# wen-yuan-zhang/MaterialRefGS

Measured on AMD Instinct MI355X. Metric: full-render fwd+bwd views/sec at 800x800/300k surfels; grad max-rel-err vs ref, higher is better.
Workload: dtype f32; 1 GPU; C3 shell scene through render_surfel: P=300000, 800x800, S=8 + deferred BRDF shading, fwd+bwd; P=300000, H=800, W=800, S=8, sh_degree=3, num_rendered=1153468, cameras_cycled=2, parallelism=single GPU, glue_epilogue=True

## Files before the change

### materialrefgs_amd/csrc/mrgs_render_bwd.hip

```cpp
#include "mrgs_blend_math.h"

#ifndef MRGS_BWD_STAGES
#define MRGS_BWD_STAGES 1
#endif


__device__ __forceinline__ void swap32_add(float& a, float b)
{
    typedef unsigned u2 __attribute__((ext_vector_type(2)));
    const u2 r = __builtin_amdgcn_permlane32_swap(__float_as_uint(a), __float_as_uint(b), false, false);
    a = __uint_as_float(r.x) + __uint_as_float(r.y);
}
__device__ __forceinline__ void swap16_add(float& a, float b)
{
    typedef unsigned u2 __attribute__((ext_vector_type(2)));
    const u2 r = __builtin_amdgcn_permlane16_swap(__float_as_uint(a), __float_as_uint(b), false, false);
    a = __uint_as_float(r.x) + __uint_as_float(r.y);
}

__device__ __forceinline__ float rows_reduce4(float a0, float a1, float a2, float a3)
{
    float t0, t1, u;
    asm volatile(
        "s_nop 1\n\t"
        "v_add_f32_dpp %0, %3, %3 row_ror:8 row_mask:0xf bank_mask:0xf\n\t"
        "v_add_f32_dpp %1, %5, %5 row_ror:8 row_mask:0xf bank_mask:0xf\n\t"
        "v_add_f32_dpp %0, %4, %4 row_ror:8 row_mask:0xf bank_mask:0xc\n\t"
        "v_add_f32_dpp %1, %6, %6 row_ror:8 row_mask:0xf bank_mask:0xc\n\t"
        "s_nop 0\n\t"
        "v_add_f32_dpp %2, %0, %0 row_half_mirror row_mask:0xf bank_mask:0xf\n\t"
        "v_add_f32_dpp %2, %1, %1 row_half_mirror row_mask:0xf bank_mask:0xa\n\t"
        "s_nop 1\n\t"
        "v_add_f32_dpp %2, %2, %2 quad_perm:[2,3,0,1] row_mask:0xf bank_mask:0xf\n\t"
        "s_nop 1\n\t"
        "v_add_f32_dpp %2, %2, %2 quad_perm:[1,0,3,2] row_mask:0xf bank_mask:0xf\n\t"
        : "=&v"(t0), "=&v"(t1), "=&v"(u)
        : "v"(a0), "v"(a1), "v"(a2), "v"(a3));
    return u;
}
__device__ __forceinline__ float rows_reduce2(float a0, float a1)
{
    float t;
    asm volatile(
        "s_nop 1\n\t"
        "v_add_f32_dpp %0, %1, %1 row_ror:8 row_mask:0xf bank_mask:0xf\n\t"
        "v_add_f32_dpp %0, %2, %2 row_ror:8 row_mask:0xf bank_mask:0xc\n\t"
        "s_nop 1\n\t"
        "v_add_f32_dpp %0, %0, %0 row_half_mirror row_mask:0xf bank_mask:0xf\n\t"
        "s_nop 1\n\t"
        "v_add_f32_dpp %0, %0, %0 quad_perm:[2,3,0,1] row_mask:0xf bank_mask:0xf\n\t"
        "s_nop 1\n\t"
        "v_add_f32_dpp %0, %0, %0 quad_perm:[1,0,3,2] row_mask:0xf bank_mask:0xf\n\t"
        : "=&v"(t)
        : "v"(a0), "v"(a1));
    return t;
}
__device__ __forceinline__ float rows_reduce1(float v)
{
    v = mrgs_dpp_add<0x128, 0xf>(v);
    v = mrgs_dpp_add<0x124, 0xf>(v);
    v = mrgs_dpp_add<0x122, 0xf>(v);
    v = mrgs_dpp_add<0x121, 0xf>(v);
    return v;
}

struct ReduceLane { uint32_t off16, off8, off4; bool w16, w8, w4; };
__device__ __forceinline__ ReduceLane mrgs_reduce_lane(int lane)
{
    const int row = lane >> 4, bank = (lane >> 2) & 3;
    const int sub = ((row & 1) << 1) | (row >> 1);
    ReduceLane r;
    r.off16 = 4u * (uint32_t)(8 * (bank & 1) + 4 * (bank >> 1) + sub);
    r.off8 = 4u * (uint32_t)(4 * (bank >> 1) + sub);
    r.off4 = 4u * (uint32_t)sub;
    r.w16 = (lane & 3) == 0;
    r.w8 = (lane & 7) == 0;
    r.w4 = (lane & 15) == 0;
    return r;
}

__device__ __forceinline__ void atomic_add_at(float* __restrict__ base, uint32_t byte_off, float v)
{
    atomicAdd((float*)((char*)base + byte_off), v);
}

template <int K>
__device__ __forceinline__ void wave_reduce_atomic_add(float (&v)[K], float* __restrict__ base, uint32_t row_off, const ReduceLane& rl)
{
    static_assert(K % 4 == 0, "pad the value count to a multiple of 4");
#pragma unroll
    for (int i = 0; i < K / 2; i++) swap32_add(v[2 * i], v[2 * i + 1]);
#pragma unroll
    for (int i = 0; i < K / 4; i++) swap16_add(v[4 * i], v[4 * i + 2]);
    constexpr int N4 = K / 4;
    constexpr int NB4 = N4 / 4;
    constexpr int REM = N4 - 4 * NB4;
#pragma unroll
    for (int t = 0; t < NB4; t++) {
        const float u = rows_reduce4(v[16 * t], v[16 * t + 4], v[16 * t + 8], v[16 * t + 12]);
        if (rl.w16) atomic_add_at(base, row_off + (64u * t + rl.off16), u);
    }
    if (REM >= 2) {
        const float u = rows_reduce2(v[16 * NB4], v[16 * NB4 + 4]);
        if (rl.w8) atomic_add_at(base, row_off + (64u * NB4 + rl.off8), u);
    }
    if (REM == 1 || REM == 3) {
        constexpr int vbase = 16 * NB4 + (REM == 3 ? 8 : 0);
        const float u = rows_reduce1(v[vbase]);
        if (rl.w4) atomic_add_at(base, row_off + (4u * vbase + rl.off4), u);
    }
}

__device__ __forceinline__ void wave_reduce_atomic_add2(float a, float b, float* __restrict__ base, uint32_t byte_off, int lane)
{
    swap32_add(a, b);
    a = rows_reduce1(a);
    a += __int_as_float(__builtin_amdgcn_update_dpp(0, __float_as_int(a), 0x142, 0xa, 0xf, false));
    if ((lane & 31) == 16) atomic_add_at(base, byte_off + 4u * (uint32_t)(lane >> 5), a);
}

__device__ __forceinline__ void wave_reduce_atomic_add1(float a, float* __restrict__ base, uint32_t byte_off, int lane)
{
    float z = 0.0f;
    swap32_add(a, z);
    a = rows_reduce1(a);
    a += __int_as_float(__builtin_amdgcn_update_dpp(0, __float_as_int(a), 0x142, 0xa, 0xf, false));
    if (lane == 16) atomic_add_at(base, byte_off, a);
}

#ifdef MRGS_WAVE_STATS
__device__ unsigned long long g_wave_stats[8 * 65536];
extern "C" int mrgs_wave_stats(unsigned long long* host, int n)
{
    return (int)hipMemcpyFromSymbol(host, HIP_SYMBOL(g_wave_stats), sizeof(unsigned long long) * n);
}
#define WS_ENTRY() const unsigned long long ws_te = wall_clock64(); unsigned long long ws_dbg[3];
#define WS_DBG , ws_dbg
#define WS_BEGIN() const unsigned long long ws_t0 = wall_clock64(), ws_c0 = __builtin_amdgcn_s_memtime(); unsigned ws_iters = 0, ws_act = 0, ws_chunks = 0;
#define WS_ITER(a) { ws_iters++; ws_act += (a) ? 1 : 0; }
#define WS_CHUNK() ws_chunks++;
#define WS_END() if (lane == 0 && b < 65536) { unsigned long long* w = g_wave_stats + 8 * (size_t)b; w[6] = ((ws_dbg[0] - ws_te) << 40) | ((ws_dbg[2] - ws_te) << 16) | ws_dbg[1]; w[7] = ws_te; w[0] = ws_t0; w[1] = wall_clock64(); \
        w[2] = __builtin_amdgcn_s_memtime() - ws_c0; w[3] = ((unsigned long long)ws_iters << 32) | ws_act; w[4] = ((unsigned long long)ws_chunks << 32) | (unsigned)max_contrib; \
        w[5] = (unsigned long long)__builtin_amdgcn_s_getreg((4 << 0) | (0 << 6) | (31 << 11)) | ((unsigned long long)__builtin_amdgcn_s_getreg((20 << 0) | (0 << 6) | (31 << 11)) << 32); }
#else
#define WS_ENTRY()
#define WS_DBG
#define WS_BEGIN()
#define WS_ITER(a)
#define WS_CHUNK()
#define WS_END()
#endif

#ifndef MRGS_BWD_WPE0
#define MRGS_BWD_WPE0 5
#endif
#ifndef MRGS_BWD_WPE8
#define MRGS_BWD_WPE8 4
#endif
template <int S_MAX, bool FV, int S_LIVE>
__global__ void __launch_bounds__(64) __attribute__((amdgpu_waves_per_eu(S_MAX == 0 ? MRGS_BWD_WPE0 : S_MAX <= 8 ? MRGS_BWD_WPE8 : 2, 8))) render_bwd_kernel(
    const uint2* __restrict__ ranges, const uint32_t* __restrict__ bwd_assign, uint32_t* __restrict__ q_bwd, const uint32_t* __restrict__ cu_state, const uint32_t* __restrict__ point_list,
    const uint8_t* __restrict__ cflag, int S, int W, int H, int tiles_x, int ntiles,
    const float4* __restrict__ rec, const float* __restrict__ features, const float* __restrict__ bg,
    const float* __restrict__ final_Ts, const uint32_t* __restrict__ n_contrib, const float* __restrict__ dL_dpixels,
    const float* __restrict__ dL_dpixels_f, const float* __restrict__ dL_dothers, float* __restrict__ grad_rec, int gstride, int slots)
{
    constexpr int SF = S_MAX > 0 ? S_MAX : 1;
    constexpr bool XREC = S_LIVE > S_MAX;
    static_assert(!XREC || (S_MAX == 8 && S_LIVE == 9 && FV), "one record channel: rows of twelve floats, eight staged");
    constexpr int S_ROW = XREC ? 12 : S_MAX;
    constexpr int S_STAGED = S_LIVE < S_MAX ? S_LIVE : S_MAX;
    constexpr int SFA = S_LIVE > SF ? S_LIVE : SF;
    constexpr int K = 16 + S_LIVE;
    constexpr int KT = K & ~3;
    __shared__ StageBuf<SF> stage[MRGS_BWD_STAGES];

    const int lane = threadIdx.x;
    const int b = blockIdx.x;
    WS_ENTRY();
    const uint32_t item = mrgs_pull_item(q_bwd, cu_state, bwd_assign, ntiles, b & 7, b >> 3, lane, slots WS_DBG);
    if (item == 0xFFFFFFFFu) return;
    const int tile = (int)((item & 0x1FFFFFFFu) >> 2), quad = (int)(item & 3u);
    const uint32_t prio = (item >> 29) & 3u;
    const uint2 range = ranges[tile];
    const int tx = tile % tiles_x, ty = tile / tiles_x;
    const int bx = tx * 2 + (quad & 1), by = ty * 2 + (quad >> 1);
    const int pxi = bx * 8 + (lane & 7), pyi = by * 8 + (lane >> 3);
    const bool inside = pxi < W && pyi < H;
    const float px = (float)pxi, py = (float)pyi;
    const int HW = H * W;
    const int pix = inside ? W * pyi + pxi : 0;

    const int last_contributor = inside ? (int)n_contrib[pix] : 0;
    int max_contrib = last_contributor;
#pragma unroll
    for (int d = 32; d >= 1; d >>= 1) max_contrib = max(max_contrib, __shfl_xor(max_contrib, d, 64));
    if (max_contrib == 0) return;
    WS_BEGIN();
    if (prio == 3u) __builtin_amdgcn_s_setprio(3);
    else if (prio == 2u) __builtin_amdgcn_s_setprio(2);
    else if (prio == 1u) __builtin_amdgcn_s_setprio(1);
    const int median_contributor = inside ? (int)n_contrib[pix + HW] : 0;

    const float T_final = inside ? final_Ts[pix] : 0.f;
    float T = T_final;
    float dL_dpixel[3] = {0.f, 0.f, 0.f};
    float dL_dpixel_f[SFA];
#pragma unroll
    for (int i = 0; i < SFA; i++) dL_dpixel_f[i] = 0.f;
    float accum_dot = 0.f;
    float dL_dreg = 0.f, dL_ddepth = 0.f, dL_daccum = 0.f, dL_dnormal2D[3] = {0.f, 0.f, 0.f}, dL_dmedian_depth = 0.f;
    if (inside && last_contributor > 0) {
        dL_ddepth = dL_dothers[0 * HW + pix];
        dL_daccum = dL_dothers[1 * HW + pix];
        dL_dnormal2D[0] = dL_dothers[2 * HW + pix];
        dL_dnormal2D[1] = dL_dothers[3 * HW + pix];
        dL_dnormal2D[2] = dL_dothers[4 * HW + pix];
        dL_dmedian_depth = dL_dothers[5 * HW + pix];
        dL_dreg = dL_dothers[6 * HW + pix];
#pragma unroll
        for (int i = 0; i < 3; i++) dL_dpixel[i] = dL_dpixels[i * HW + pix];
        if (S_MAX > 0) {
#pragma unroll
            for (int i = 0; i < S_LIVE; i++)
                if (i < S) dL_dpixel_f[i] = dL_dpixels_f[(size_t)i * HW + pix];
        }
    }
    const float final_D = inside ? final_Ts[pix + HW] : 0.f;
    const float final_D2 = inside ? final_Ts[pix + 2 * HW] : 0.f;
    const float mscale = MRGS_FAR_N / (MRGS_FAR_N - MRGS_NEAR_N);
    const float dmd_scale = (MRGS_FAR_N * MRGS_NEAR_N) / (MRGS_FAR_N - MRGS_NEAR_N);
    const float bg_dot_dpixel = fmaf(bg[2], dL_dpixel[2], fmaf(bg[1], dL_dpixel[1], bg[0] * dL_dpixel[0]));

    const uint32_t* plist = point_list + range.x;
    const uint8_t* qm = cflag + (size_t)range.x * 4 + quad;
    const ReduceLane rl = mrgs_reduce_lane(lane);
    const uint32_t row_bytes = (uint32_t)gstride * 4u;
    const int c_top = (max_contrib - 1) / MRGS_CHUNK;
    uint32_t idq1 = 0, idq2 = 0;
    uint64_t mask_cur, exact_cur;
    {
        uint32_t id0 = 0, q0 = 0;
        if (c_top * MRGS_CHUNK + lane < max_contrib) { id0 = plist[c_top * MRGS_CHUNK + lane]; q0 = qm[(size_t)(c_top * MRGS_CHUNK + lane) * 4]; }
        if (c_top >= 1) idq1 = plist[(c_top - 1) * MRGS_CHUNK + lane] | ((uint32_t)qm[(size_t)((c_top - 1) * MRGS_CHUNK + lane) * 4] << 28);
        if (c_top >= 2) idq2 = plist[(c_top - 2) * MRGS_CHUNK + lane] | ((uint32_t)qm[(size_t)((c_top - 2) * MRGS_CHUNK + lane) * 4] << 28);
        const bool cand0 = q0 & 1u;
        mask_cur = __builtin_amdgcn_ballot_w64(cand0);
        exact_cur = __builtin_amdgcn_ballot_w64((q0 & 2u) != 0u);
        mrgs_stage_async<S_MAX, SF, FV, S_LIVE, S_ROW>(stage[c_top % MRGS_BWD_STAGES], rec, features, S, id0, cand0);
        if (cand0) stage[c_top % MRGS_BWD_STAGES].id[lane] = id0 * row_bytes;
    }

    for (int c = c_top; c >= 0; c--) {
        const int base = c * MRGS_CHUNK;
        mrgs_stage_wait();
        WS_CHUNK();
        uint64_t mask_nxt = 0ull, exact_nxt = 0ull;
        auto stage_next = [&]() {
            const bool cand1 = (idq1 >> 28) & 1u;
            exact_nxt = __builtin_amdgcn_ballot_w64(((idq1 >> 29) & 1u) != 0u);
            const uint32_t id1 = idq1 & 0x0FFFFFFFu;
            mask_nxt = __builtin_amdgcn_ballot_w64(cand1);
            mrgs_stage_async<S_MAX, SF, FV, S_LIVE, S_ROW>(stage[(c + 1) % MRGS_BWD_STAGES], rec, features, S, id1, cand1);
            if (cand1) stage[(c + 1) % MRGS_BWD_STAGES].id[lane] = id1 * row_bytes;
            idq1 = idq2;
            idq2 = 0;
            if (c >= 3) idq2 = plist[(c - 3) * MRGS_CHUNK + lane] | ((uint32_t)qm[(size_t)((c - 3) * MRGS_CHUNK + lane) * 4] << 28);
        };
        if (MRGS_BWD_STAGES == 2) stage_next();

        uint64_t mask = mask_cur;
        const uint64_t exact_mask = exact_cur;
        const StageBuf<SF>& sb = stage[c % MRGS_BWD_STAGES];

        auto blend_entry = [&](const SurfelGeom& sg, int j) {
            const int contributor = base + j;
            Hit h;
            bool active;
            active = mrgs_intersect(sg, px, py, h) & !(h.depth < MRGS_NEAR_LO);
            if (__builtin_expect((exact_mask >> j) & 1ull, 0)) active = mrgs_intersect_exact<true>(sg, px, py, h);
            active = active & inside & (contributor < last_contributor);
            const uint64_t amask = __builtin_amdgcn_ballot_w64(active);
            WS_ITER(amask != 0ull);
            if (amask == 0ull) return;
            const bool use3d = h.use3d;
            const bool a3 = active & use3d;
            const float4 a0 = sb.rec[3][j], a1 = sb.rec[4][j];
            const float normal[3] = {a0.x, a0.y, a0.z};
            const float col[3] = {a0.w, a1.x, a1.y};
            const float alpha = active ? h.alpha : 0.0f;
            const float G = active ? h.G : 0.0f;
            const float c_d = active ? h.depth : 1.0f;
            const float sx = a3 ? h.sx : 0.0f, sy = a3 ? h.sy : 0.0f;
            const float inv_pz = a3 ? h.inv_pz : 0.0f;

            float g[K];
            const float inv_1ma = mrgs_rcp(1.0f - alpha);
            T = T * inv_1ma;
            const float w = alpha * T;
            const float one_m_a = 1.0f - alpha;
            float q = 0.0f;
#pragma unroll
            for (int ch = 0; ch < 3; ch++) {
                q = fmaf(col[ch], dL_dpixel[ch], q);
                g[MRGS_G_COL + ch] = w * dL_dpixel[ch];
            }
            if (S_MAX > 0) {
#pragma unroll
                for (int ch = 0; ch < S_STAGED; ch++) {
                    const float f = (FV || ch < S) ? mrgs_staged_feature<FV>(sb, ch, j) : 0.0f;
                    q = fmaf(f, dL_dpixel_f[ch], q);
                    g[MRGS_G_FEAT + ch] = w * dL_dpixel_f[ch];
                }
                if (XREC) {
                    q = fmaf(a1.w, dL_dpixel_f[S_MAX], q);
                    g[MRGS_G_FEAT + S_MAX] = w * dL_dpixel_f[S_MAX];
                }
            }
#pragma unroll
            for (int ch = 0; ch < 3; ch++) {
                q = fmaf(normal[ch], dL_dnormal2D[ch], q);
                g[MRGS_G_NRM + ch] = w * dL_dnormal2D[ch];
            }
            const float inv_cd = mrgs_rcp(c_d);
            const float m_d = mscale * (1.0f - MRGS_NEAR_N * inv_cd);
            const float dmd_dd = dmd_scale * inv_cd * inv_cd;
            float dL_dz = (active & (contributor == median_contributor - 1)) ? dL_dmedian_depth : 0.0f;
            const float final_A = 1.0f - T_final;
            const float dL_dweight = fmaf(-2.0f * m_d, final_D, fmaf(m_d * m_d, final_A, final_D2)) * dL_dreg;
            const float dL_dmd = 2.0f * w * fmaf(m_d, final_A, -final_D) * dL_dreg;
            dL_dz = fmaf(dL_dmd, dmd_dd, dL_dz);
            q = fmaf(c_d, dL_ddepth, q);
            q += dL_daccum;
            q += dL_dweight;
            float dL_dalpha = q - accum_dot;
            accum_dot = fmaf(alpha, q, one_m_a * accum_dot);
            dL_dalpha *= T;
            dL_dalpha = fmaf(-T_final * inv_1ma, bg_dot_dpixel, dL_dalpha);
            dL_dalpha = active ? dL_dalpha : 0.0f;
            const float dL_dG = sg.g2.w * dL_dalpha;
            dL_dz = fmaf(w, dL_ddepth, dL_dz);
            {
                const float Twx = sg.g1.z, Twy = sg.g1.w;
                const float dGn = dL_dG * -G;
                const float dL_dsx = fmaf(dGn, sx, dL_dz * Twx);
                const float dL_dsy = fmaf(dGn, sy, dL_dz * Twy);
                const float dpx = dL_dsx * inv_pz, dpy = dL_dsy * inv_pz;
                const float dpz = -fmaf(dpx, sx, dpy * sy);
                const float ndkx = fmaf(-h.ly, dpz, h.lz * dpy);
                const float ndky = fmaf(-h.lz, dpx, h.lx * dpz);
                const float ndkz = fmaf(-h.lx, dpy, h.ly * dpx);
                const float ndlx = fmaf(-dpy, h.kz, dpz * h.ky);
                const float ndly = fmaf(-dpz, h.kx, dpx * h.kz);
                const float ndlz = fmaf(-dpx, h.ky, dpy * h.kx);
                g[0] = ndkx; g[1] = ndky; g[2] = ndkz;
                g[3] = ndlx; g[4] = ndly; g[5] = ndlz;
                g[6] = fmaf(px, -ndkx, fmaf(py, -ndlx, dL_dz * sx));
                g[7] = fmaf(px, -ndky, fmaf(py, -ndly, dL_dz * sy));
                g[8] = fmaf(px, -ndkz, fmaf(py, -ndlz, dL_dz));
            }
            g[MRGS_G_OPA] = G * dL_dalpha;
            const uint32_t row_off = sb.id[j];
            if constexpr (KT == K) {
                wave_reduce_atomic_add<K>(g, grad_rec, row_off, rl);
            } else {
                float gt[KT];
#pragma unroll
                for (int k = 0; k < KT; k++) gt[k] = g[k];
                wave_reduce_atomic_add<KT>(gt, grad_rec, row_off, rl);
#pragma unroll
                for (int k = KT; k < K; k++) wave_reduce_atomic_add1(g[k], grad_rec, row_off + 4u * (uint32_t)k, lane);
            }
            const bool a2 = active & !use3d;
            if (__builtin_amdgcn_ballot_w64(a2) != 0ull) {
                const float dL_dG2 = a2 ? dL_dG : 0.0f;
                const float dGf = -G * MRGS_FILTER_INV_SQUARE;
                wave_reduce_atomic_add2(dL_dG2 * (dGf * h.dx), dL_dG2 * (dGf * h.dy), grad_rec, row_off + 4u * MRGS_G_M2(S_ROW), lane);
            }
        };

        if (mask != 0ull) {
            int j = 63 - __builtin_clzll(mask);
            SurfelGeom sA, sB;
            sA.g0 = sb.rec[0][j]; sA.g1 = sb.rec[1][j]; sA.g2 = sb.rec[2][j];
            while (true) {
                mask &= ~(1ull << j);
                bool more = mask != 0ull;
                int jn = more ? 63 - __builtin_clzll(mask) : j;
                sB.g0 = sb.rec[0][jn]; sB.g1 = sb.rec[1][jn]; sB.g2 = sb.rec[2][jn];
                blend_entry(sA, j);
                if (!more) break;
                j = jn;
                mask &= ~(1ull << j);
                more = mask != 0ull;
                jn = more ? 63 - __builtin_clzll(mask) : j;
                sA.g0 = sb.rec[0][jn]; sA.g1 = sb.rec[1][jn]; sA.g2 = sb.rec[2][jn];
                blend_entry(sB, j);
                if (!more) break;
                j = jn;
            }
        }
        if (MRGS_BWD_STAGES == 1) stage_next();
        mask_cur = mask_nxt;
        exact_cur = exact_nxt;
    }
    mrgs_stage_wait();
    WS_END();
}

#define MRGS_BWD_KERNEL render_bwd_kernel

void mrgs_launch_render_bwd(const MrgsRasterConfig& cfg, const MrgsRasterInputs& in, const MrgsGeomWs& g, const uint32_t* plist,
                            const uint8_t* cflag, const MrgsImgWs& img, const float* dL_dpix, const float* dL_dpix_f, const float* dL_dothers,
                            float* grad_rec, bool forward_queues, hipStream_t stream)
{
    const uint32_t* assign = forward_queues ? img.fwd_assign : img.bwd_assign;
    const int tiles_x = (cfg.W + MRGS_BLOCK_X - 1) / MRGS_BLOCK_X, tiles_y = (cfg.H + MRGS_BLOCK_Y - 1) / MRGS_BLOCK_Y;
    const int ntiles = tiles_x * tiles_y;
    const int nblocks = (((ntiles + 7) / 8) * 4 + MRGS_MAX_SIMD_QUEUES) * 8;
    const dim3 grid(nblocks), block(64);
#define LAUNCH(GS, SM, ...)                                                                                                       \
    hipLaunchKernelGGL((MRGS_BWD_KERNEL<SM, __VA_ARGS__>), grid, block, 0, stream, img.ranges, assign, img.q_bwd, img.blend_state + MRGS_CS_BASE, plist, cflag, cfg.S, cfg.W, cfg.H, tiles_x, ntiles, \
                       g.rec, in.features, in.bg, img.final_T, img.n_contrib, dL_dpix, dL_dpix_f, dL_dothers, grad_rec, GS, mrgs_waves_per_simd<MRGS_BWD_KERNEL<SM, __VA_ARGS__>>())
    const int gs = MRGS_GRAD_STRIDE(cfg.S);
    const bool fv_ok = ((uintptr_t)in.features & 15u) == 0;
    if (cfg.S == 0) LAUNCH(gs, 0, false, 0);
    else if (cfg.S == 8 && fv_ok) LAUNCH(gs, 8, true, 8);
    else if (cfg.S <= 8) LAUNCH(gs, 8, false, 8);
    else if (cfg.S == 12 && fv_ok && in.features_live == 9u) LAUNCH(gs, 8, true, 9);
    else if (cfg.S == 12 && fv_ok) LAUNCH(gs, 12, true, 12);
    else if (cfg.S <= 12) LAUNCH(gs, 12, false, 12);
    else if (cfg.S == 24 && fv_ok) LAUNCH(gs, 24, true, 24);
    else LAUNCH(gs, 24, false, 24);
#undef LAUNCH
}
```

Before: 1198 views/s.

## Compute color/feature/normal gradient sums via MFMA over batched surfels

For the S=8 feature-vector path, the per-surfel gradients that are w times a per-pixel constant (normals, colors, features) are no longer reduced across the wave with DPP shuffles. Instead, each surfel's per-pixel weights are buffered in LDS in batches of eight, and the sums are computed as a small matrix product with 16x16x4 f32 MFMA against the per-pixel dL vectors. The products are then atomically added to the gradient rows. This cuts the number of cross-lane reductions per surfel, at the cost of extra LDS traffic, wave barriers, reuse of the stage buffer for the C matrix, and a different summation order.

```diff
diff --git a/materialrefgs_amd/csrc/mrgs_render_bwd.hip b/materialrefgs_amd/csrc/mrgs_render_bwd.hip
--- a/materialrefgs_amd/csrc/mrgs_render_bwd.hip
+++ b/materialrefgs_amd/csrc/mrgs_render_bwd.hip
@@ -119,14 +119,12 @@
     if ((lane & 31) == 16) atomic_add_at(base, byte_off + 4u * (uint32_t)(lane >> 5), a);
 }
 
-__device__ __forceinline__ void wave_reduce_atomic_add1(float a, float* __restrict__ base, uint32_t byte_off, int lane)
-{
-    float z = 0.0f;
-    swap32_add(a, z);
-    a = rows_reduce1(a);
-    a += __int_as_float(__builtin_amdgcn_update_dpp(0, __float_as_int(a), 0x142, 0xa, 0xf, false));
-    if (lane == 16) atomic_add_at(base, byte_off, a);
-}
+#define MRGS_MS_SLOTS 8
+#define MRGS_MS_WROW 68
+#define MRGS_MS_CROW 17
+typedef float mrgs_f32x4 __attribute__((ext_vector_type(4)));
+template <int S_MAX, bool FV, int S_LIVE>
+constexpr bool mrgs_bwd_matrix_sums = S_MAX == 8 && S_LIVE <= 9 && FV;
 
 #ifdef MRGS_WAVE_STATS
 __device__ unsigned long long g_wave_stats[8 * 65536];
@@ -171,9 +169,15 @@
     constexpr int S_ROW = XREC ? 12 : S_MAX;
     constexpr int S_STAGED = S_LIVE < S_MAX ? S_LIVE : S_MAX;
     constexpr int SFA = S_LIVE > SF ? S_LIVE : SF;
-    constexpr int K = 16 + S_LIVE;
-    constexpr int KT = K & ~3;
+    constexpr bool MS = mrgs_bwd_matrix_sums<S_MAX, FV, S_LIVE>;
+    constexpr int MS_COLS = 6 + S_LIVE;
+    constexpr int K = MS ? 10 : 16 + S_LIVE;
+    static_assert(MS || K % 4 == 0, "whole groups of four through the transposing reduction");
+    static_assert(!MS || (MS_COLS <= 16 && MRGS_G_COL == MRGS_G_NRM + 3 && MRGS_G_FEAT == MRGS_G_COL + 3), "one 16-wide tile of contiguous floats");
     __shared__ StageBuf<SF> stage[MRGS_BWD_STAGES];
+    __shared__ __attribute__((aligned(16))) float ms_w[MS ? MRGS_MS_SLOTS * MRGS_MS_WROW : 1];
+    __shared__ __attribute__((aligned(16))) uint32_t ms_row[MS ? MRGS_MS_SLOTS : 1];
+    static_assert(!MS || sizeof(StageBuf<SF>) >= sizeof(float) * 64 * MRGS_MS_CROW, "C passes through the stage buffer");
 
     const int lane = threadIdx.x;
     const int b = blockIdx.x;
@@ -231,6 +235,56 @@
     const float mscale = MRGS_FAR_N / (MRGS_FAR_N - MRGS_NEAR_N);
     const float dmd_scale = (MRGS_FAR_N * MRGS_NEAR_N) / (MRGS_FAR_N - MRGS_NEAR_N);
     const float bg_dot_dpixel = fmaf(bg[2], dL_dpixel[2], fmaf(bg[1], dL_dpixel[1], bg[0] * dL_dpixel[0]));
+
+    float ms_c[MS ? 16 : 1];
+    if constexpr (MS) {
+        float* cbuf = reinterpret_cast<float*>(&stage[0]);
+        float* cw = cbuf + MRGS_MS_CROW * lane;
+#pragma unroll
+        for (int i = 0; i < 3; i++) { cw[i] = dL_dnormal2D[i]; cw[3 + i] = dL_dpixel[i]; }
+#pragma unroll
+        for (int i = 0; i < S_LIVE; i++) cw[6 + i] = dL_dpixel_f[i];
+#pragma unroll
+        for (int i = MS_COLS; i < 16; i++) cw[i] = 0.0f;
+        __builtin_amdgcn_fence(__ATOMIC_RELEASE, "wavefront");
+        __builtin_amdgcn_wave_barrier();
+        __builtin_amdgcn_fence(__ATOMIC_ACQUIRE, "wavefront");
+        const float* cr = cbuf + MRGS_MS_CROW * 16 * (lane >> 4) + (lane & 15);
+#pragma unroll
+        for (int s = 0; s < 16; s++) ms_c[s] = cr[MRGS_MS_CROW * s];
+        asm volatile("s_waitcnt lgkmcnt(0)" ::: "memory");
+        __builtin_amdgcn_wave_barrier();
+    }
+    int ms_n = 0;
+    auto ms_flush = [&]() {
+        if constexpr (MS) {
+            __builtin_amdgcn_fence(__ATOMIC_RELEASE, "wavefront");
+            __builtin_amdgcn_wave_barrier();
+            __builtin_amdgcn_fence(__ATOMIC_ACQUIRE, "wavefront");
+            const mrgs_f32x4* wr = reinterpret_cast<const mrgs_f32x4*>(ms_w + MRGS_MS_WROW * (lane & 7) + 16 * (lane >> 4));
+            const uint4 ro = *reinterpret_cast<const uint4*>(ms_row + 4 * ((lane >> 4) & 1));
+            mrgs_f32x4 acc0 = {0.0f, 0.0f, 0.0f, 0.0f}, acc1 = {0.0f, 0.0f, 0.0f, 0.0f};
+            mrgs_f32x4 a[4];
+#pragma unroll
+            for (int t = 0; t < 4; t++) a[t] = wr[t];
+            __builtin_amdgcn_sched_barrier(0);
+#pragma unroll
+            for (int t = 0; t < 4; t++) {
+                acc0 = __builtin_amdgcn_mfma_f32_16x16x4f32(a[t][0], ms_c[4 * t + 0], acc0, 0, 0, 0);
+                acc1 = __builtin_amdgcn_mfma_f32_16x16x4f32(a[t][1], ms_c[4 * t + 1], acc1, 0, 0, 0);
+                acc0 = __builtin_amdgcn_mfma_f32_16x16x4f32(a[t][2], ms_c[4 * t + 2], acc0, 0, 0, 0);
+                acc1 = __builtin_amdgcn_mfma_f32_16x16x4f32(a[t][3], ms_c[4 * t + 3], acc1, 0, 0, 0);
+            }
+            const int e0 = 4 * (lane >> 4);
+            const uint32_t col_off = 4u * (uint32_t)(MRGS_G_NRM + (lane & 15));
+            const bool col_live = lane < 32 && (lane & 15) < MS_COLS;
+            const uint32_t roff[4] = {ro.x, ro.y, ro.z, ro.w};
+#pragma unroll
+            for (int r = 0; r < 4; r++)
+                if (col_live && e0 + r < ms_n) atomic_add_at(grad_rec, roff[r] + col_off, acc0[r] + acc1[r]);
+            ms_n = 0;
+        }
+    };
 
     const uint32_t* plist = point_list + range.x;
     const uint8_t* qm = cflag + (size_t)range.x * 4 + quad;
@@ -303,24 +357,21 @@
 #pragma unroll
             for (int ch = 0; ch < 3; ch++) {
                 q = fmaf(col[ch], dL_dpixel[ch], q);
-                g[MRGS_G_COL + ch] = w * dL_dpixel[ch];
+                if constexpr (!MS) g[MRGS_G_COL + ch] = w * dL_dpixel[ch];
             }
             if (S_MAX > 0) {
 #pragma unroll
                 for (int ch = 0; ch < S_STAGED; ch++) {
                     const float f = (FV || ch < S) ? mrgs_staged_feature<FV>(sb, ch, j) : 0.0f;
                     q = fmaf(f, dL_dpixel_f[ch], q);
-                    g[MRGS_G_FEAT + ch] = w * dL_dpixel_f[ch];
+                    if constexpr (!MS) g[MRGS_G_FEAT + ch] = w * dL_dpixel_f[ch];
                 }
-                if (XREC) {
-                    q = fmaf(a1.w, dL_dpixel_f[S_MAX], q);
-                    g[MRGS_G_FEAT + S_MAX] = w * dL_dpixel_f[S_MAX];
-                }
+                if (XREC) q = fmaf(a1.w, dL_dpixel_f[S_MAX], q);
             }
 #pragma unroll
             for (int ch = 0; ch < 3; ch++) {
                 q = fmaf(normal[ch], dL_dnormal2D[ch], q);
-                g[MRGS_G_NRM + ch] = w * dL_dnormal2D[ch];
+                if constexpr (!MS) g[MRGS_G_NRM + ch] = w * dL_dnormal2D[ch];
             }
             const float inv_cd = mrgs_rcp(c_d);
             const float m_d = mscale * (1.0f - MRGS_NEAR_N * inv_cd);
@@ -361,21 +412,27 @@
             }
             g[MRGS_G_OPA] = G * dL_dalpha;
             const uint32_t row_off = sb.id[j];
-            if constexpr (KT == K) {
+            if constexpr (MS) {
+                ms_w[MRGS_MS_WROW * ms_n + lane] = w;
+                if (lane == 0) ms_row[ms_n] = row_off;
+                ms_n++;
+                float gt[8];
+#pragma unroll
+                for (int k = 0; k < 8; k++) gt[k] = g[k];
+                wave_reduce_atomic_add<8>(gt, grad_rec, row_off, rl);
+                static_assert(MRGS_G_OPA == 9, "the pair (dL/dT[8], opacity) is contiguous");
+                wave_reduce_atomic_add2(g[8], g[MRGS_G_OPA], grad_rec, row_off + 4u * 8u, lane);
+            } else {
                 wave_reduce_atomic_add<K>(g, grad_rec, row_off, rl);
-            } else {
-                float gt[KT];
-#pragma unroll
-                for (int k = 0; k < KT; k++) gt[k] = g[k];
-                wave_reduce_atomic_add<KT>(gt, grad_rec, row_off, rl);
-#pragma unroll
-                for (int k = KT; k < K; k++) wave_reduce_atomic_add1(g[k], grad_rec, row_off + 4u * (uint32_t)k, lane);
             }
             const bool a2 = active & !use3d;
             if (__builtin_amdgcn_ballot_w64(a2) != 0ull) {
                 const float dL_dG2 = a2 ? dL_dG : 0.0f;
                 const float dGf = -G * MRGS_FILTER_INV_SQUARE;
                 wave_reduce_atomic_add2(dL_dG2 * (dGf * h.dx), dL_dG2 * (dGf * h.dy), grad_rec, row_off + 4u * MRGS_G_M2(S_ROW), lane);
+            }
+            if constexpr (MS) {
+                if (ms_n == MRGS_MS_SLOTS) ms_flush();
             }
         };
 
@@ -404,6 +461,9 @@
         mask_cur = mask_nxt;
         exact_cur = exact_nxt;
     }
+    if constexpr (MS) {
+        if (ms_n > 0) ms_flush();
+    }
     mrgs_stage_wait();
     WS_END();
 }
```

Result: slower. 1180 views/s (-1.5%).
